# howardlau1999/pytorch-ddp-template

Hardware: AMD Instinct MI355X
Metric: samples/sec (whole node) ResNet-18/CIFAR-shape DDP (higher is better)
Workload: dtype bf16; 1 GPU; model=resnet18-cifar, global_batch=8192, image=32, num_classes=10, parallelism=dp1, hip_graph=True, optimizer=sgd+momentum(master fp32)

## Files before the change

pytorch_ddp_template_amd/ops/csrc/conv_glds.hip:

```cpp

#include <torch/extension.h>

#include "common.h"
#include "dispatch.h"

namespace cg {

typedef __bf16 bf16x8 __attribute__((ext_vector_type(8)));
typedef float f32x4 __attribute__((ext_vector_type(4)));

constexpr int BM = 256, BK = 64;
constexpr int THREADS = 512;

__device__ __forceinline__ f32x4 mfma16(bf16x8 a, bf16x8 b, f32x4 c) {
  return __builtin_amdgcn_mfma_f32_16x16x32_bf16(a, b, c, 0, 0, 0);
}

__device__ __forceinline__ int kswz(int row, int kbyte) {
  return kbyte ^ (((row >> 2) & 1) << 5);
}

struct Geom {
  int H, W, C, lgC, HO, WO, stride, pad, S, RS;
  int lgSt = 0;
};

constexpr int EPI_NONE = 0, EPI_ADD = 1, EPI_MASK = 2, EPI_ADD_MASK = 3;
constexpr int EPI_BNSTATS = 4, EPI_MASK_BNSTATS = EPI_MASK | EPI_BNSTATS;

constexpr int halo_pitch(int hw) { return (hw + 2 + 7) & ~7; }
constexpr int halo_bytes(int hw) {
  return hw ? (BM / hw + 2) * halo_pitch(hw) * BK * 2 : 0;
}

template <int BN, bool STATS, int EPI = EPI_NONE, int HW = 0>
__global__ __launch_bounds__(THREADS, HW ? 4 : BN == 64 ? 2 : 1)
void conv_fwd_glds_kernel(
    const __hip_bfloat16* __restrict__ x, const __hip_bfloat16* __restrict__ w,
    __hip_bfloat16* __restrict__ y, const __hip_bfloat16* __restrict__ zpad,
    int M, int N , int K , Geom g,
    float* __restrict__ stats_ws, int ws_nblocks,
    const __hip_bfloat16* __restrict__ addend,
    const __hip_bfloat16* __restrict__ out_mask,
    const float* __restrict__ bn_mean, const float* __restrict__ bn_rstd) {
  static_assert(!(STATS && EPI != EPI_NONE),
                "dgrad epilogues carry no forward stats");
  static_assert(!(EPI & EPI_BNSTATS) || EPI == EPI_MASK_BNSTATS,
                "BN-backward sums ride only with the mask, without an addend");
  static_assert(HW == 0 || (BN == 64 && BM % HW == 0 && HW % 16 == 0),
                "halo variant: 64-wide tile, whole image rows per M-tile");
  constexpr int HALO_ELEMS = halo_bytes(HW) / 2;
  __shared__ __hip_bfloat16
      smem[HW ? HALO_ELEMS + 2 * BN * BK : 2 * (BM + BN) * BK];

  const int tid = threadIdx.x;
  const int lane = tid & 63;
  const int wave = tid >> 6;

  long long nwg = (long long)gridDim.x * gridDim.y;
  long long bid = (long long)blockIdx.y * gridDim.x + blockIdx.x;
  {
    const long long q = nwg >> 3, r = nwg & 7;
    const int xcd = (int)(bid & 7);
    const long long o = bid >> 3;
    bid = (xcd < r ? xcd * (q + 1) : r * (q + 1) + (xcd - r) * q) + o;
  }
  const int n0 = (int)(bid % gridDim.x) * BN;
  const long long m0 = (bid / gridDim.x) * BM;
  const long long flat_id = bid;

  const int srow = (tid >> 3) & 7;
  const int schunk = lane & 7;
  constexpr int RA = BM / 64;
  constexpr int RB = BN / 64;

  long long nbase[RA];
  int hv[RA], wv[RA];
#pragma unroll
  for (int r = 0; r < RA; ++r) {
    const long long m = m0 + r * 64 + wave * 8 + srow;
    const int wo = (int)(m % g.WO);
    const long long t = m / g.WO;
    const int ho = (int)(t % g.HO);
    const long long n = t / g.HO;
    hv[r] = ho * g.stride - g.pad;
    wv[r] = wo * g.stride - g.pad;
    nbase[r] = n * g.H * (long long)g.W;
  }
  const int smask = (1 << g.lgSt) - 1;

  auto stage = [&](int buf, int kt) {
    __hip_bfloat16* sa = smem + buf * ((BM + BN) * BK);
    __hip_bfloat16* sb = sa + BM * BK;
    const int tap = (kt << 6) >> g.lgC;
    const int c0 = (kt << 6) & (g.C - 1);
    const int rt = tap / g.S, st = tap - rt * g.S;
#pragma unroll
    for (int r = 0; r < RA; ++r) {
      const int row = r * 64 + wave * 8 + srow;
      const int kk = c0 + kswz(row, schunk * 16) / 2;
      const __hip_bfloat16* src = zpad;
      const int hs = hv[r] + rt, ws = wv[r] + st;
      if ((unsigned)(hs >> g.lgSt) < (unsigned)g.H &&
          (unsigned)(ws >> g.lgSt) < (unsigned)g.W &&
          ((hs | ws) & smask) == 0)
        src = x + ((nbase[r] + (long long)(hs >> g.lgSt) * g.W +
                    (ws >> g.lgSt))
                   << g.lgC) +
              kk;
      __builtin_amdgcn_global_load_lds(
          (const __attribute__((address_space(1))) unsigned int*)src,
          (__attribute__((address_space(3))) unsigned int*)(
              sa + (r * 64 + wave * 8) * BK),
          16, 0, 0);
    }
#pragma unroll
    for (int r = 0; r < RB; ++r) {
      const int row = r * 64 + wave * 8 + srow;
      const long long kk = (long long)kt * BK + kswz(row, schunk * 16) / 2;
      __builtin_amdgcn_global_load_lds(
          (const __attribute__((address_space(1))) unsigned int*)(
              w + (long long)(n0 + row) * K + kk),
          (__attribute__((address_space(3))) unsigned int*)(
              sb + (r * 64 + wave * 8) * BK),
          16, 0, 0);
    }
  };

  constexpr int NWM = BM / 128;
  constexpr int NWN = 8 / NWM;
  constexpr int NI = BN / (16 * NWN);
  const int wm = (wave / NWN) * 128;
  const int wn = (wave % NWN) * (NI * 16);
  const int frow = lane & 15;
  const int fkb = (lane >> 4) * 16;

  f32x4 acc[8][NI];
#pragma unroll
  for (int i = 0; i < 8; ++i)
#pragma unroll
    for (int j = 0; j < NI; ++j) acc[i][j] = f32x4{0.f, 0.f, 0.f, 0.f};

  if constexpr (HW == 0) {
    const int NT = K / BK;
    stage(0, 0);
    __syncthreads();

    int cur = 0;
    for (int kt = 0; kt < NT; ++kt) {
      if (kt + 1 < NT) stage(cur ^ 1, kt + 1);
      const __hip_bfloat16* sa = smem + cur * ((BM + BN) * BK);
      const __hip_bfloat16* sb = sa + BM * BK;
      bf16x8 bf[NI][2];
#pragma unroll
      for (int ni = 0; ni < NI; ++ni)
#pragma unroll
        for (int ks = 0; ks < 2; ++ks) {
          const int row = wn + ni * 16 + frow;
          bf[ni][ks] = *(const bf16x8*)((const char*)(sb + row * BK) +
                                        kswz(row, ks * 64 + fkb));
        }
#pragma unroll
      for (int mi = 0; mi < 8; ++mi) {
        bf16x8 af[2];
#pragma unroll
        for (int ks = 0; ks < 2; ++ks) {
          const int row = wm + mi * 16 + frow;
          af[ks] = *(const bf16x8*)((const char*)(sa + row * BK) +
                                    kswz(row, ks * 64 + fkb));
        }
#pragma unroll
        for (int ni = 0; ni < NI; ++ni) {
          acc[mi][ni] = mfma16(af[0], bf[ni][0], acc[mi][ni]);
          acc[mi][ni] = mfma16(af[1], bf[ni][1], acc[mi][ni]);
        }
      }
      __syncthreads();
      cur ^= 1;
    }
  } else {
    constexpr int HP = halo_pitch(HW);
    constexpr int KR = BM / HW;
    constexpr int PPR = HP / 8;
    constexpr int NPIECE = (KR + 2) * PPR;
    __hip_bfloat16* sw = smem + HALO_ELEMS;
    const int tpi = g.H / KR;
    const int tile = (int)(m0 / BM);
    const long long img = tile / tpi;
    const int h0 = (tile - (int)img * tpi) * KR;

    auto stage_w = [&](int buf, int kt) {
      __hip_bfloat16* sb = sw + buf * (BN * BK);
#pragma unroll
      for (int r = 0; r < RB; ++r) {
        const int row = r * 64 + wave * 8 + srow;
        const long long kk = (long long)kt * BK + kswz(row, schunk * 16) / 2;
        __builtin_amdgcn_global_load_lds(
            (const __attribute__((address_space(1))) unsigned int*)(
                w + (long long)(n0 + row) * K + kk),
            (__attribute__((address_space(3))) unsigned int*)(
                sb + (r * 64 + wave * 8) * BK),
            16, 0, 0);
      }
    };
    stage_w(0, 0);
#pragma unroll
    for (int p0 = 0; p0 < NPIECE; p0 += 8) {
      const int pc = p0 + wave;
      if (pc < NPIECE) {
        const int hr = pc / PPR;
        const int hi = h0 - 1 + hr;
        const int wi = (pc - hr * PPR) * 8 + (lane & 7) - 1;
        const __hip_bfloat16* src = zpad;
        if ((unsigned)hi < (unsigned)g.H && (unsigned)wi < (unsigned)HW)
          src = x + (((img * g.H + hi) * HW + wi) << 6) + (lane >> 3) * 8;
        __builtin_amdgcn_global_load_lds(
            (const __attribute__((address_space(1))) unsigned int*)src,
            (__attribute__((address_space(3))) unsigned int*)(smem + pc * 512),
            16, 0, 0);
      }
    }
    int abase[3];
#pragma unroll
    for (int st = 0; st < 3; ++st) {
      const int q = frow + st;
      abase[st] = (wm / HW) * HP * 128 + (q >> 3) * 1024 + (q & 7) * 16 +
                  (lane >> 4) * 128;
    }
    __syncthreads();

#pragma unroll 1
    for (int rt = 0; rt < 3; ++rt)
#pragma unroll
    for (int st = 0; st < 3; ++st) {
      const int kt = rt * 3 + st;
      if (kt + 1 < 9) stage_w((kt + 1) & 1, kt + 1);
      const __hip_bfloat16* sb = sw + (kt & 1) * (BN * BK);
      const char* ha = (const char*)smem + rt * (HP * 128) + abase[st];
      bf16x8 bf[NI][2];
#pragma unroll
      for (int ni = 0; ni < NI; ++ni)
#pragma unroll
        for (int ks = 0; ks < 2; ++ks) {
          const int row = wn + ni * 16 + frow;
          bf[ni][ks] = *(const bf16x8*)((const char*)(sb + row * BK) +
                                        kswz(row, ks * 64 + fkb));
        }
#pragma unroll
      for (int mi = 0; mi < 8; ++mi) {
        const int cpos = ((mi * 16) / HW) * HP + (mi * 16) % HW;
        bf16x8 af[2];
#pragma unroll
        for (int ks = 0; ks < 2; ++ks)
          af[ks] = *(const bf16x8*)(ha + cpos * 128 + ks * 512);
#pragma unroll
        for (int ni = 0; ni < NI; ++ni) {
          acc[mi][ni] = mfma16(af[0], bf[ni][0], acc[mi][ni]);
          acc[mi][ni] = mfma16(af[1], bf[ni][1], acc[mi][ni]);
        }
      }
      __syncthreads();
    }
  }

  if (STATS && stats_ws) {
#pragma unroll
    for (int ni = 0; ni < NI; ++ni) {
      float sv = 0.f, qv = 0.f;
#pragma unroll
      for (int mi = 0; mi < 8; ++mi)
#pragma unroll
        for (int reg = 0; reg < 4; ++reg) {
          const float v = acc[mi][ni][reg];
          sv += v;
          qv += v * v;
        }
      sv += __shfl_xor(sv, 16);
      qv += __shfl_xor(qv, 16);
      sv += __shfl_xor(sv, 32);
      qv += __shfl_xor(qv, 32);
      if (lane < 16) {
        const int col = n0 + wn + ni * 16 + frow;
        const long long wsrow =
            ((flat_id * NWM + wave / NWN)) % ws_nblocks;
        atomicAdd(&stats_ws[wsrow * N + col], sv);
        atomicAdd(&stats_ws[((long long)ws_nblocks + wsrow) * N + col], qv);
      }
    }
  }

  __hip_bfloat16* cs = smem;
  constexpr int CPR = BN / 8;
  constexpr int RPR = THREADS / CPR;
  constexpr int NR = BM / RPR;
  const int wrow = tid / CPR, wchunk = tid % CPR;
  constexpr bool HAS_ADD = (EPI & EPI_ADD) != 0;
  constexpr bool HAS_MASK = (EPI & EPI_MASK) != 0;
  constexpr bool HAS_BNS = (EPI & EPI_BNSTATS) != 0;
  constexpr int PF = 2;
  static_assert(NR >= PF, "epilogue prefetch deeper than the store loop");
  short8 av[PF] = {}, mv[PF] = {};
  auto epi_load = [&](int r, int slot) {
    const long long off =
        ((m0 + r * RPR + wrow) * N + n0) * 2 + wchunk * 16;
    if constexpr (HAS_ADD || HAS_BNS)
      av[slot] = *(const short8*)((const char*)addend + off);
    if constexpr (HAS_MASK)
      mv[slot] = *(const short8*)((const char*)out_mask + off);
  };
  if constexpr (EPI != EPI_NONE) {
#pragma unroll
    for (int p = 0; p < PF; ++p) epi_load(p, p);
  }
#pragma unroll
  for (int mi = 0; mi < 8; ++mi)
#pragma unroll
    for (int ni = 0; ni < NI; ++ni) {
      const int col = wn + ni * 16 + frow;
#pragma unroll
      for (int reg = 0; reg < 4; ++reg) {
        const int row = wm + mi * 16 + (lane >> 4) * 4 + reg;
        cs[row * BN + col] = f2bf(acc[mi][ni][reg]);
      }
    }
  float mu[8] = {}, rs[8] = {}, sdg[8] = {}, sdb[8] = {};
  if constexpr (HAS_BNS) {
#pragma unroll
    for (int j = 0; j < 8; ++j) {
      mu[j] = bn_mean[n0 + wchunk * 8 + j];
      rs[j] = bn_rstd[n0 + wchunk * 8 + j];
    }
  }
  __syncthreads();
  if constexpr (!HAS_BNS) {
#pragma unroll
    for (int r = 0; r < NR; ++r) {
      const int row = r * RPR + wrow;
      short8 c = *(const short8*)((const char*)(cs + row * BN) + wchunk * 16);
      if constexpr (EPI != EPI_NONE) {
        const short8 a = av[r % PF], m = mv[r % PF];
        if (r + PF < NR) epi_load(r + PF, r % PF);
#pragma unroll
        for (int j = 0; j < 8; ++j) {
          short v = c[j];
          if constexpr (HAS_ADD) v = f2bfbits(bfbits2f(v) + bfbits2f(a[j]));
          if constexpr (HAS_MASK)
            v = f2bfbits(bfbits2f(m[j]) > 0.f ? bfbits2f(v) : 0.f);
          c[j] = v;
        }
      }
      *(short8*)((char*)(y + (m0 + row) * N + n0) + wchunk * 16) = c;
    }
  } else {
    static_assert(PF == 2 && NR % PF == 0, "store loop steps by slot pairs");
    auto store_round = [&](int r, int slot) {
      const int row = r * RPR + wrow;
      short8 c = *(const short8*)((const char*)(cs + row * BN) + wchunk * 16);
      const short8 t = av[slot], m = mv[slot];
      if (r + PF < NR) epi_load(r + PF, slot);
#pragma unroll
      for (int j = 0; j < 8; ++j) {
        const float gv = bfbits2f(m[j]) > 0.f ? bfbits2f(c[j]) : 0.f;
        c[j] = f2bfbits(gv);
        sdb[j] += gv;
        sdg[j] += gv * (bfbits2f(t[j]) - mu[j]) * rs[j];
      }
      *(short8*)((char*)(y + (m0 + row) * N + n0) + wchunk * 16) = c;
    };
#pragma unroll 1
    for (int r = 0; r < NR; r += PF) {
      store_round(r, 0);
      store_round(r + 1, 1);
    }
  }

  if constexpr (HAS_BNS) {
    constexpr int P = THREADS / (2 * BN);
    constexpr int RP = RPR / P;
    static_assert(P >= 1 && RP * P == RPR, "column reduction split");
    static_assert((2 * RPR * BN + P * 2 * BN) * sizeof(float) <=
                      sizeof(smem), "reduction buffers exceed the tile LDS");
    float* red = reinterpret_cast<float*>(smem);
    float* red2 = red + 2 * RPR * BN;
    __syncthreads();
#pragma unroll
    for (int j = 0; j < 8; ++j) {
      red[wrow * BN + wchunk * 8 + j] = sdg[j];
      red[(RPR + wrow) * BN + wchunk * 8 + j] = sdb[j];
    }
    __syncthreads();
    const int ci = tid % (2 * BN), part = tid / (2 * BN);
    const int which = ci / BN, col = ci % BN;
    float s = 0.f;
#pragma unroll
    for (int i = 0; i < RP; ++i)
      s += red[(which * RPR + part * RP + i) * BN + col];
    if constexpr (P > 1) {
      red2[part * 2 * BN + ci] = s;
      __syncthreads();
      if (part != 0) return;
      s = red2[ci];
#pragma unroll
      for (int p = 1; p < P; ++p) s += red2[p * 2 * BN + ci];
    }
    const long long wsrow = flat_id % ws_nblocks;
    atomicAdd(&stats_ws[((long long)which * ws_nblocks + wsrow) * N + n0 + col],
              s);
  }
}

}

struct GldsBnStats {
  const torch::Tensor& bn_x;
  const torch::Tensor& mean;
  const torch::Tensor& rstd;
  torch::Tensor ws;
};

constexpr int kBnStatsRows = 1024;

bool conv_halo64_eligible(int64_t H, int64_t W, int64_t C, int64_t Kout,
                          int64_t R, int64_t S, int64_t stride, int64_t pad) {
  if (R != 3 || S != 3 || stride != 1 || pad != 1 || C != 64) return false;
  if (Kout <= 0 || Kout % 64 || Kout % 128 == 0) return false;
  if (W < 16 || W % 16 || cg::BM % W) return false;
  const int64_t k = cg::BM / W;
  if (k > H || H % k) return false;
  return cg::halo_bytes((int)W) + 2 * 64 * cg::BK * 2 <=
         2 * (cg::BM + 64) * cg::BK * 2;
}

static bool conv2d_glds_launch(const torch::Tensor& x, const torch::Tensor& w,
                               torch::Tensor& y, const torch::Tensor& zp,
                               int64_t stride, int64_t pad, float* stats_ws,
                               int ws_nblocks, int lgSt,
                               const c10::optional<torch::Tensor>& addend,
                               const c10::optional<torch::Tensor>& out_mask,
                               GldsBnStats* bns) {
  static const char* e = getenv("PDT_CONV_GLDS");
  if (e && e[0] == '0') return false;
  if (x.scalar_type() != torch::kBFloat16) return false;
  const int N_ = (int)x.size(0), H = (int)x.size(1), W = (int)x.size(2),
            C = (int)x.size(3);
  const int Kout = (int)w.size(0), R = (int)w.size(1), S = (int)w.size(2);
  if (C < 64 || (C & (C - 1))) return false;
  const int HO = (int)y.size(1), WO = (int)y.size(2);
  const int lgC = log2_exact(C);
  const long long M = (long long)N_ * HO * WO;
  const int K = R * S * C;
  if (Kout % 64) return false;
  const int BN = Kout % 256 == 0 ? 256 : Kout % 128 == 0 ? 128 : 64;
  if (M % cg::BM) return false;
  if (M / cg::BM > 2147483647LL / 8) return false;
  cg::Geom g{H, W, C, lgC, HO, WO, (int)stride, (int)pad, S, R * S, lgSt};
  auto stream = c10::hip::getCurrentHIPStream();
  dim3 grid(Kout / BN, (unsigned)(M / cg::BM));
  const int epi = (addend.has_value() ? cg::EPI_ADD : 0) |
                  (out_mask.has_value() ? cg::EPI_MASK : 0);
  for (const auto* t : {&addend, &out_mask}) {
    if (!t->has_value()) continue;
    TORCH_CHECK(!stats_ws,
                "conv glds: addend/out_mask exclude the stats epilogue");
    TORCH_CHECK((*t)->is_cuda() && (*t)->is_contiguous() &&
                    (*t)->scalar_type() == x.scalar_type() &&
                    (*t)->numel() == y.numel(),
                "conv glds: addend/out_mask must be contiguous, of dy's dtype "
                "and dx-sized");
  }
  const bf16* addp = addend.has_value() ? ptr16<bf16>(*addend) : nullptr;
  const bf16* maskp = out_mask.has_value() ? ptr16<bf16>(*out_mask) : nullptr;
  const float *meanp = nullptr, *rstdp = nullptr;
  if (bns) {
    TORCH_CHECK(epi == cg::EPI_MASK && !stats_ws,
                "conv glds: BN-backward sums need out_mask and no addend");
    TORCH_CHECK(bns->bn_x.is_cuda() && bns->bn_x.is_contiguous() &&
                    bns->bn_x.scalar_type() == x.scalar_type() &&
                    bns->bn_x.numel() == y.numel(),
                "conv glds: bn_x must be contiguous, of dy's dtype and "
                "dx-sized");
    for (const auto* t : {&bns->mean, &bns->rstd})
      TORCH_CHECK(t->is_cuda() && t->is_contiguous() &&
                      t->scalar_type() == torch::kFloat32 &&
                      t->numel() == Kout,
                  "conv glds: bn_mean/bn_rstd must be fp32 [C]");
    ws_nblocks = (int)std::min<long long>(kBnStatsRows,
                                          (long long)grid.x * grid.y);
    bns->ws = torch::zeros({2LL * ws_nblocks, Kout},
                           x.options().dtype(torch::kFloat32));
    stats_ws = bns->ws.data_ptr<float>();
    addp = ptr16<bf16>(bns->bn_x);
    meanp = bns->mean.data_ptr<float>();
    rstdp = bns->rstd.data_ptr<float>();
  }
  const char* eh = getenv("PDT_CONV_HALO64");
  const bool halo = !(eh && eh[0] == '0') && lgSt == 0 && H == HO && W == WO &&
                    conv_halo64_eligible(H, W, C, Kout, R, S, stride, pad);
#define CG_HALO(ST, EP)                                       \
  (W == 16   ? &cg::conv_fwd_glds_kernel<64, ST, EP, 16>      \
   : W == 32 ? &cg::conv_fwd_glds_kernel<64, ST, EP, 32>      \
             : &cg::conv_fwd_glds_kernel<64, ST, EP, 64>)
#define CG_KERN(ST, EP)                                       \
  (halo        ? CG_HALO(ST, EP)                              \
   : BN == 256 ? &cg::conv_fwd_glds_kernel<256, ST, EP>       \
   : BN == 128 ? &cg::conv_fwd_glds_kernel<128, ST, EP>       \
               : &cg::conv_fwd_glds_kernel<64, ST, EP>)
  auto kern = bns                     ? CG_KERN(false, cg::EPI_MASK_BNSTATS)
              : stats_ws              ? CG_KERN(true, cg::EPI_NONE)
              : epi == cg::EPI_NONE   ? CG_KERN(false, cg::EPI_NONE)
              : epi == cg::EPI_ADD    ? CG_KERN(false, cg::EPI_ADD)
              : epi == cg::EPI_MASK   ? CG_KERN(false, cg::EPI_MASK)
                                      : CG_KERN(false, cg::EPI_ADD_MASK);
#undef CG_KERN
#undef CG_HALO
  hipLaunchKernelGGL(kern, grid, dim3(cg::THREADS), 0, stream, ptr16<bf16>(x),
                     ptr16<bf16>(w), ptr16<bf16>(y), ptr16<bf16>(zp), (int)M,
                     Kout, K, g, stats_ws, ws_nblocks, addp, maskp, meanp,
                     rstdp);
  return true;
}

bool conv2d_fwd_glds_ex(const torch::Tensor& x, const torch::Tensor& w,
                        torch::Tensor& y, const torch::Tensor& zp,
                        int64_t stride, int64_t pad, float* stats_ws,
                        int ws_nblocks, int lgSt,
                        const c10::optional<torch::Tensor>& addend,
                        const c10::optional<torch::Tensor>& out_mask) {
  return conv2d_glds_launch(x, w, y, zp, stride, pad, stats_ws, ws_nblocks,
                            lgSt, addend, out_mask, nullptr);
}

torch::Tensor conv2d_dgrad_glds_bnstats(
    const torch::Tensor& dy, const torch::Tensor& wr, torch::Tensor& dx,
    const torch::Tensor& zp, int64_t pad, int lgSt,
    const torch::Tensor& out_mask, const torch::Tensor& bn_x,
    const torch::Tensor& bn_mean, const torch::Tensor& bn_rstd) {
  GldsBnStats bns{bn_x, bn_mean, bn_rstd, torch::Tensor()};
  if (!conv2d_glds_launch(dy, wr, dx, zp, 1, pad, nullptr, 0, lgSt,
                          c10::nullopt, out_mask, &bns))
    return torch::Tensor();
  return bns.ws;
}

bool conv2d_fwd_glds(const torch::Tensor& x, const torch::Tensor& w,
                     torch::Tensor& y, const torch::Tensor& zp,
                     int64_t stride, int64_t pad, float* stats_ws,
                     int ws_nblocks) {
  return conv2d_fwd_glds_ex(x, w, y, zp, stride, pad, stats_ws, ws_nblocks,
                            0, c10::nullopt, c10::nullopt);
}
```

pytorch_ddp_template_amd/ops/csrc/ops.cpp:

```cpp

#include <torch/extension.h>

#include <vector>

torch::Tensor relu_fwd(torch::Tensor x);
torch::Tensor relu_bwd(torch::Tensor dy, torch::Tensor y);
torch::Tensor add_relu_fwd(torch::Tensor a, torch::Tensor b);
torch::Tensor add_(torch::Tensor a, torch::Tensor b);
torch::Tensor gelu_fwd(torch::Tensor x);
torch::Tensor gelu_bwd(torch::Tensor dy, torch::Tensor x);
torch::Tensor col_sum(torch::Tensor dy);
torch::Tensor transpose2d(torch::Tensor x);
torch::Tensor avgpool_global(torch::Tensor x);
torch::Tensor avgpool_global_bwd(torch::Tensor dy, int64_t H, int64_t W);
std::vector<torch::Tensor> maxpool2d_fwd(torch::Tensor x, int64_t k, int64_t s,
                                         int64_t p);
torch::Tensor maxpool2d_bwd(torch::Tensor dy, torch::Tensor idx, int64_t H,
                            int64_t W);
torch::Tensor weight_rot(torch::Tensor w);
torch::Tensor zero_stuff(torch::Tensor dy, int64_t s, int64_t opad_h,
                         int64_t opad_w);
torch::Tensor im2col(torch::Tensor x, int64_t R, int64_t S, int64_t stride,
                     int64_t pad, int64_t Kpad);
torch::Tensor bmm_nt_bf16(torch::Tensor A, torch::Tensor B,
                          c10::optional<torch::Tensor> bias, bool relu);
torch::Tensor gemm_nt_splitk_f32(torch::Tensor A, torch::Tensor B);
torch::Tensor bmm_tn_bf16(torch::Tensor A, torch::Tensor B);
std::vector<torch::Tensor> bmm_tn_bias_bf16(torch::Tensor A, torch::Tensor B);
torch::Tensor conv2d_fwd_bf16(torch::Tensor x, torch::Tensor w,
                              c10::optional<torch::Tensor> bias, int64_t stride,
                              int64_t pad, bool relu);
torch::Tensor conv2d_wgrad_bf16(torch::Tensor dy, torch::Tensor x,
                                int64_t stride, int64_t pad, int64_t R,
                                int64_t S);
torch::Tensor conv2d_dgrad_bf16(torch::Tensor dy, torch::Tensor wr,
                                int64_t stride, int64_t pad, int64_t H,
                                int64_t W,
                                c10::optional<torch::Tensor> addend,
                                c10::optional<torch::Tensor> addend_mask,
                                c10::optional<torch::Tensor> out_mask);
std::vector<torch::Tensor> conv2d_fwd_stats_bf16(
    torch::Tensor x, torch::Tensor w, c10::optional<torch::Tensor> bias,
    int64_t stride, int64_t pad, bool relu);
std::vector<torch::Tensor> conv2d_dgrad_bnstats_bf16(
    torch::Tensor dy, torch::Tensor wr, int64_t stride, int64_t pad, int64_t H,
    int64_t W, torch::Tensor out_mask, torch::Tensor bn_x,
    torch::Tensor bn_mean, torch::Tensor bn_rstd);
bool conv_halo64_eligible(int64_t H, int64_t W, int64_t C, int64_t Kout,
                          int64_t R, int64_t S, int64_t stride, int64_t pad);
torch::Tensor bmm_nt_f32(torch::Tensor A, torch::Tensor B,
                         c10::optional<torch::Tensor> bias, bool relu);
torch::Tensor bmm_tn_f32(torch::Tensor A, torch::Tensor B);
torch::Tensor conv2d_fwd_f32(torch::Tensor x, torch::Tensor w,
                             c10::optional<torch::Tensor> bias, int64_t stride,
                             int64_t pad, bool relu);
torch::Tensor conv2d_wgrad_f32(torch::Tensor dy, torch::Tensor x,
                               int64_t stride, int64_t pad, int64_t R,
                               int64_t S);
std::vector<torch::Tensor> bn_fwd(torch::Tensor x, torch::Tensor gamma,
                                  torch::Tensor beta,
                                  c10::optional<torch::Tensor> running_mean,
                                  c10::optional<torch::Tensor> running_var,
                                  double momentum, double eps, bool relu);
std::vector<torch::Tensor> bn_fwd_ws(torch::Tensor x, torch::Tensor gamma,
                                     torch::Tensor beta, torch::Tensor ws,
                                     c10::optional<torch::Tensor> running_mean,
                                     c10::optional<torch::Tensor> running_var,
                                     double momentum, double eps, bool relu,
                                     c10::optional<torch::Tensor> addend);
torch::Tensor bn_infer(torch::Tensor x, torch::Tensor gamma, torch::Tensor beta,
                       torch::Tensor rmean, torch::Tensor rvar, double eps,
                       bool relu);
std::vector<torch::Tensor> bn_bwd(torch::Tensor dy, torch::Tensor x,
                                  torch::Tensor gamma, torch::Tensor mean,
                                  torch::Tensor rstd,
                                  c10::optional<torch::Tensor> y_relu);
std::vector<torch::Tensor> bn_bwd_ws(torch::Tensor dy, torch::Tensor x,
                                     torch::Tensor gamma, torch::Tensor mean,
                                     torch::Tensor rstd, torch::Tensor ws);
std::vector<torch::Tensor> layernorm_fwd(torch::Tensor x, torch::Tensor gamma,
                                         torch::Tensor beta, double eps);
std::vector<torch::Tensor> layernorm_bwd(torch::Tensor dy, torch::Tensor x,
                                         torch::Tensor gamma,
                                         torch::Tensor mean,
                                         torch::Tensor rstd);
torch::Tensor softmax_fwd(torch::Tensor x, double scale);
torch::Tensor softmax_bwd(torch::Tensor dy, torch::Tensor y, double scale);
std::vector<torch::Tensor> ce_fwd(torch::Tensor logits, torch::Tensor target);
torch::Tensor ce_bwd(torch::Tensor logits, torch::Tensor target,
                     torch::Tensor lse, torch::Tensor dloss);
torch::Tensor mse_fwd(torch::Tensor p, torch::Tensor t);
torch::Tensor mse_bwd(torch::Tensor p, torch::Tensor t, torch::Tensor dloss);
std::vector<torch::Tensor> qkv_unpack(torch::Tensor qkv, int64_t heads);
torch::Tensor qkv_pack(torch::Tensor dq, torch::Tensor dk, torch::Tensor dv,
                       int64_t N, int64_t heads);
torch::Tensor head_split(torch::Tensor x, int64_t heads);
std::vector<torch::Tensor> attn_fwd(torch::Tensor qkv, int64_t heads,
                                    double scale, bool want_p);
torch::Tensor attn_bwd(torch::Tensor qkv, torch::Tensor dout,
                       torch::Tensor out, torch::Tensor stats, int64_t heads,
                       double scale);
void sgd_step(std::vector<torch::Tensor> params,
              std::vector<torch::Tensor> grads,
              std::vector<torch::Tensor> moms,
              std::vector<torch::Tensor> masters, double lr, double momentum,
              double wd, double damp, bool nesterov,
              c10::optional<torch::Tensor> guard,
              c10::optional<torch::Tensor> skip_count,
              c10::optional<torch::Tensor> lr_tensor);
torch::Tensor l2norm_sq(std::vector<torch::Tensor> grads);
void scale_(std::vector<torch::Tensor> ts, double s);
void scale_by_tensor_(std::vector<torch::Tensor> ts, torch::Tensor s);


namespace {

bool is_bf16(const torch::Tensor& t) {
  return t.scalar_type() == torch::kBFloat16 ||
         t.scalar_type() == torch::kHalf;
}

int k_granule(const torch::Tensor& t) { return is_bf16(t) ? 8 : 4; }

torch::Tensor pad_k(const torch::Tensor& t, int mult) {
  long long K = t.size(-1);
  long long pad = (mult - K % mult) % mult;
  if (pad == 0) return t;
  return torch::constant_pad_nd(t, {0, pad});
}

bool pow2_ge(int v, int lo) {
  return v >= lo && (v & (v - 1)) == 0;
}

}

torch::Tensor gemm_nt(torch::Tensor A, torch::Tensor B,
                      c10::optional<torch::Tensor> bias, bool relu,
                      bool ) {
  TORCH_CHECK(A.scalar_type() == B.scalar_type(), "dtype mismatch");
  int g = k_granule(A);
  if (A.size(-1) % g) {
    A = pad_k(A.contiguous(), g);
    B = pad_k(B.contiguous(), g);
  }
  if (is_bf16(A)) return bmm_nt_bf16(A.contiguous(), B.contiguous(), bias, relu);
  return bmm_nt_f32(A.contiguous(), B.contiguous(), bias, relu);
}

torch::Tensor gemm_tn(torch::Tensor A, torch::Tensor B) {
  if (is_bf16(A)) return bmm_tn_bf16(A.contiguous(), B.contiguous());
  return bmm_tn_f32(A.contiguous(), B.contiguous());
}

torch::Tensor bmm_nt(torch::Tensor A, torch::Tensor B) {
  int g = k_granule(A);
  if (A.size(-1) % g) {
    A = pad_k(A.contiguous(), g);
    B = pad_k(B.contiguous(), g);
  }
  if (is_bf16(A)) return bmm_nt_bf16(A.contiguous(), B.contiguous(), {}, false);
  return bmm_nt_f32(A.contiguous(), B.contiguous(), {}, false);
}

torch::Tensor bmm_tn(torch::Tensor A, torch::Tensor B) {
  auto C = is_bf16(A) ? bmm_tn_bf16(A.contiguous(), B.contiguous())
                      : bmm_tn_f32(A.contiguous(), B.contiguous());
  return C.to(A.scalar_type());
}

torch::Tensor bmm_nn(torch::Tensor A, torch::Tensor B) {
  auto Bt = transpose2d(B.contiguous());
  return bmm_nt(A, Bt);
}


torch::Tensor conv2d_fwd(torch::Tensor x, torch::Tensor w,
                         c10::optional<torch::Tensor> bias, int64_t stride,
                         int64_t pad, bool relu) {
  int Cin = (int)x.size(3);
  int R = (int)w.size(1), S = (int)w.size(2), Kout = (int)w.size(0);
  const bool fast = is_bf16(x) ? pow2_ge(Cin, 8) : pow2_ge(Cin, 4);
  if (fast) {
    if (is_bf16(x))
      return conv2d_fwd_bf16(x.contiguous(), w.contiguous(), bias, stride, pad,
                             relu);
    return conv2d_fwd_f32(x.contiguous(), w.contiguous(), bias, stride, pad,
                          relu);
  }
  int K = R * S * Cin;
  int g = k_granule(x);
  int Kpad = (K + g - 1) / g * g;
  auto cols = im2col(x.contiguous(), R, S, stride, pad, Kpad);
  auto wf = pad_k(w.contiguous().reshape({Kout, K}), g);
  auto y = is_bf16(x) ? bmm_nt_bf16(cols, wf.contiguous(), bias, relu)
                      : bmm_nt_f32(cols, wf.contiguous(), bias, relu);
  int N = (int)x.size(0), H = (int)x.size(1), W = (int)x.size(2);
  int HO = (H + 2 * (int)pad - R) / (int)stride + 1;
  int WO = (W + 2 * (int)pad - S) / (int)stride + 1;
  return y.reshape({N, HO, WO, Kout});
}

torch::Tensor conv2d_dgrad(torch::Tensor dy, torch::Tensor w, int64_t stride,
                           int64_t pad, int64_t H, int64_t W,
                           c10::optional<torch::Tensor> addend,
                           c10::optional<torch::Tensor> addend_mask,
                           c10::optional<torch::Tensor> out_mask) {
  int R = (int)w.size(1), S = (int)w.size(2);
  TORCH_CHECK(pad <= R - 1 && pad <= S - 1, "dgrad needs pad <= kernel-1");
  auto wr = weight_rot(w.contiguous());
  int Kout = (int)dy.size(3);
  if (is_bf16(dy) ? pow2_ge(Kout, 8) : false) {
    return conv2d_dgrad_bf16(dy.contiguous(), wr, stride, pad, H, W, addend,
                             addend_mask, out_mask);
  }
  int64_t opad_h = (H + 2 * pad - R) % stride;
  int64_t opad_w = (W + 2 * pad - S) % stride;
  auto dys = stride > 1 ? zero_stuff(dy.contiguous(), stride, opad_h, opad_w)
                        : dy.contiguous();
  auto dx = conv2d_fwd(dys, wr, {}, 1, R - 1 - pad, false);
  if (addend.has_value()) {
    auto a = *addend;
    if (addend_mask.has_value())
      a = a * (addend_mask->reshape(a.sizes()) > 0).to(a.scalar_type());
    dx = dx + a.reshape(dx.sizes());
  }
  if (out_mask.has_value())
    dx = torch::where(out_mask->reshape(dx.sizes()) > 0, dx,
                      torch::zeros_like(dx));
  TORCH_CHECK(dx.size(1) == H && dx.size(2) == W,
              "dgrad shape mismatch: got ", dx.sizes(), " want H=", H, " W=",
              W, " (input H+2p-R must be divisible by stride)");
  return dx;
}

std::tuple<torch::Tensor, c10::optional<torch::Tensor>> conv2d_dgrad_bnstats(
    torch::Tensor dy, torch::Tensor w, int64_t stride, int64_t pad, int64_t H,
    int64_t W, torch::Tensor out_mask, torch::Tensor bn_x,
    torch::Tensor bn_mean, torch::Tensor bn_rstd) {
  int R = (int)w.size(1), S = (int)w.size(2);
  TORCH_CHECK(pad <= R - 1 && pad <= S - 1, "dgrad needs pad <= kernel-1");
  if (is_bf16(dy) && pow2_ge((int)dy.size(3), 8)) {
    auto wr = weight_rot(w.contiguous());
    auto r = conv2d_dgrad_bnstats_bf16(dy.contiguous(), wr, stride, pad, H, W,
                                       out_mask, bn_x, bn_mean, bn_rstd);
    if (r.size() == 2) return {r[0], r[1]};
    return {r[0], c10::nullopt};
  }
  return {conv2d_dgrad(dy, w, stride, pad, H, W, c10::nullopt, c10::nullopt,
                       out_mask),
          c10::nullopt};
}

torch::Tensor conv2d_wgrad(torch::Tensor dy, torch::Tensor x, int64_t stride,
                           int64_t pad, int64_t R, int64_t S) {
  int Cin = (int)x.size(3);
  const bool fast = is_bf16(x) ? pow2_ge(Cin, 8) : pow2_ge(Cin, 4);
  dy = dy.contiguous();
  x = x.contiguous();
  if (fast) {
    return is_bf16(x) ? conv2d_wgrad_bf16(dy, x, stride, pad, R, S)
                      : conv2d_wgrad_f32(dy, x, stride, pad, R, S);
  }
  int K = (int)(R * S * Cin);
  int g = k_granule(x);
  int Kpad = (K + g - 1) / g * g;
  auto cols = im2col(x, R, S, stride, pad, Kpad);
  int Kout = (int)dy.size(3);
  auto dw = is_bf16(x)
                ? bmm_tn_bf16(dy.reshape({-1, Kout}).contiguous(), cols)
                : bmm_tn_f32(dy.reshape({-1, Kout}).contiguous(), cols);
  return dw.narrow(1, 0, K).reshape({Kout, R, S, Cin}).contiguous();
}

PYBIND11_MODULE(TORCH_EXTENSION_NAME, m) {
  m.def("gemm_nt", &gemm_nt, py::arg("A"), py::arg("B"),
        py::arg("bias") = c10::nullopt, py::arg("relu") = false,
        py::arg("out_f32") = false);
  m.def("gemm_tn", &gemm_tn);
  m.def("gemm_nt_splitk_f32", &gemm_nt_splitk_f32);
  m.def("gemm_tn_bias", [](torch::Tensor A, torch::Tensor B) {
    TORCH_CHECK(A.scalar_type() == torch::kBFloat16 ||
                A.scalar_type() == torch::kHalf,
                "gemm_tn_bias: 16-bit dtypes only");
    return bmm_tn_bias_bf16(A.contiguous(), B.contiguous());
  });
  m.def("bmm_nt", &bmm_nt);
  m.def("bmm_nn", &bmm_nn);
  m.def("bmm_tn", &bmm_tn);
  m.def("transpose2d", &transpose2d);
  m.def("conv2d_fwd", &conv2d_fwd, py::arg("x"), py::arg("w"),
        py::arg("bias") = c10::nullopt, py::arg("stride") = 1,
        py::arg("pad") = 0, py::arg("relu") = false);
  m.def("conv2d_dgrad", &conv2d_dgrad, py::arg("dy"), py::arg("w"),
        py::arg("stride"), py::arg("pad"), py::arg("H"), py::arg("W"),
        py::arg("addend") = c10::nullopt,
        py::arg("addend_mask") = c10::nullopt,
        py::arg("out_mask") = c10::nullopt);
  m.def("conv2d_dgrad_bnstats", &conv2d_dgrad_bnstats, py::arg("dy"),
        py::arg("w"), py::arg("stride"), py::arg("pad"), py::arg("H"),
        py::arg("W"), py::arg("out_mask"), py::arg("bn_x"),
        py::arg("bn_mean"), py::arg("bn_rstd"));
  m.def("conv2d_fwd_stats", &conv2d_fwd_stats_bf16, py::arg("x"),
        py::arg("w"), py::arg("bias") = c10::nullopt, py::arg("stride") = 1,
        py::arg("pad") = 0, py::arg("relu") = false);
  m.def("conv_halo64_eligible", &conv_halo64_eligible, py::arg("H"),
        py::arg("W"), py::arg("C"), py::arg("Kout"), py::arg("R"),
        py::arg("S"), py::arg("stride"), py::arg("pad"));
  m.def("conv2d_wgrad", &conv2d_wgrad);
  m.def("relu_fwd", &relu_fwd);
  m.def("relu_bwd", &relu_bwd);
  m.def("add_relu_fwd", &add_relu_fwd);
  m.def("add_", &add_);
  m.def("gelu_fwd", &gelu_fwd);
  m.def("gelu_bwd", &gelu_bwd);
  m.def("col_sum", &col_sum);
  m.def("avgpool_global", &avgpool_global);
  m.def("avgpool_global_bwd", &avgpool_global_bwd);
  m.def("maxpool2d_fwd", &maxpool2d_fwd);
  m.def("maxpool2d_bwd", &maxpool2d_bwd);
  m.def("bn_fwd", &bn_fwd);
  m.def("bn_fwd_ws", &bn_fwd_ws, py::arg("x"), py::arg("gamma"),
        py::arg("beta"), py::arg("ws"), py::arg("running_mean"),
        py::arg("running_var"), py::arg("momentum"), py::arg("eps"),
        py::arg("relu"), py::arg("addend") = c10::nullopt);
  m.def("bn_infer", &bn_infer);
  m.def("bn_bwd", &bn_bwd, py::arg("dy"), py::arg("x"), py::arg("gamma"),
        py::arg("mean"), py::arg("rstd"), py::arg("y_relu") = c10::nullopt);
  m.def("bn_bwd_ws", &bn_bwd_ws, py::arg("dy"), py::arg("x"),
        py::arg("gamma"), py::arg("mean"), py::arg("rstd"), py::arg("ws"));
  m.def("layernorm_fwd", &layernorm_fwd);
  m.def("layernorm_bwd", &layernorm_bwd);
  m.def("softmax_fwd", &softmax_fwd);
  m.def("attn_fwd", &attn_fwd, py::arg("qkv"), py::arg("heads"),
        py::arg("scale"), py::arg("want_p") = false);
  m.def("attn_bwd", &attn_bwd);
  m.def("qkv_unpack", &qkv_unpack);
  m.def("qkv_pack", &qkv_pack);
  m.def("head_split", &head_split);
  m.def("softmax_bwd", &softmax_bwd);
  m.def("ce_fwd", &ce_fwd);
  m.def("ce_bwd", &ce_bwd);
  m.def("mse_fwd", &mse_fwd);
  m.def("mse_bwd", &mse_bwd);
  m.def("sgd_step", &sgd_step, py::arg("params"), py::arg("grads"),
        py::arg("moms"), py::arg("masters"), py::arg("lr"),
        py::arg("momentum"), py::arg("wd"), py::arg("damp"),
        py::arg("nesterov"), py::arg("guard") = py::none(),
        py::arg("skip_count") = py::none(),
        py::arg("lr_tensor") = py::none());
  m.def("l2norm_sq", &l2norm_sq);
  m.def("scale_", &scale_);
  m.def("scale_by_tensor_", &scale_by_tensor_);
  m.def("im2col", &im2col);
  m.def("weight_rot", &weight_rot);
  m.def("zero_stuff", &zero_stuff);
}
```

Baseline: 143,200 samples/sec.

## Split stride-2 dgrad into output-parity classes to skip zero-dilated taps

Adds a parity-split variant of the implicit-GEMM conv kernel for the data-gradient of 3x3 stride-2 convolutions. Each M-tile handles one (row, column) output parity class and gathers only the 1, 2 or 4 taps that touch real (non-dilated) input, instead of iterating all 9 taps and loading zero padding for most of them. Output rows are scattered back to interleaved positions in the epilogue. This cuts wasted MFMA and load work by roughly half or more for stride-2 dgrad layers. The cost is load imbalance across parity tiles and strided epilogue stores. It is enabled by default and can be turned off with an env var.

```diff
diff --git a/pytorch_ddp_template_amd/ops/csrc/conv_glds.hip b/pytorch_ddp_template_amd/ops/csrc/conv_glds.hip
--- a/pytorch_ddp_template_amd/ops/csrc/conv_glds.hip
+++ b/pytorch_ddp_template_amd/ops/csrc/conv_glds.hip
@@ -33,7 +33,7 @@
   return hw ? (BM / hw + 2) * halo_pitch(hw) * BK * 2 : 0;
 }
 
-template <int BN, bool STATS, int EPI = EPI_NONE, int HW = 0>
+template <int BN, bool STATS, int EPI = EPI_NONE, int HW = 0, bool PAR = false>
 __global__ __launch_bounds__(THREADS, HW ? 4 : BN == 64 ? 2 : 1)
 void conv_fwd_glds_kernel(
     const __hip_bfloat16* __restrict__ x, const __hip_bfloat16* __restrict__ w,
@@ -49,6 +49,8 @@
                 "BN-backward sums ride only with the mask, without an addend");
   static_assert(HW == 0 || (BN == 64 && BM % HW == 0 && HW % 16 == 0),
                 "halo variant: 64-wide tile, whole image rows per M-tile");
+  static_assert(!PAR || (!STATS && HW == 0),
+                "parity split: dgrad only, per-tap gather");
   constexpr int HALO_ELEMS = halo_bytes(HW) / 2;
   __shared__ __hip_bfloat16
       smem[HW ? HALO_ELEMS + 2 * BN * BK : 2 * (BM + BN) * BK];
@@ -66,7 +68,11 @@
     bid = (xcd < r ? xcd * (q + 1) : r * (q + 1) + (xcd - r) * q) + o;
   }
   const int n0 = (int)(bid % gridDim.x) * BN;
-  const long long m0 = (bid / gridDim.x) * BM;
+  const long long mtile = bid / gridDim.x;
+  const int pa = PAR ? (int)(mtile >> 1) & 1 : 0;
+  const int pb = PAR ? (int)mtile & 1 : 0;
+  const long long m0 = (PAR ? mtile >> 2 : mtile) * BM;
+  const int lgH = PAR ? 31 - __clz(g.H) : 0, lgW = PAR ? 31 - __clz(g.W) : 0;
   const long long flat_id = bid;
 
   const int srow = (tid >> 3) & 7;
@@ -79,6 +85,12 @@
 #pragma unroll
   for (int r = 0; r < RA; ++r) {
     const long long m = m0 + r * 64 + wave * 8 + srow;
+    if constexpr (PAR) {
+      hv[r] = (int)(m >> lgW) & (g.H - 1);
+      wv[r] = (int)m & (g.W - 1);
+      nbase[r] = m;
+      continue;
+    }
     const int wo = (int)(m % g.WO);
     const long long t = m / g.WO;
     const int ho = (int)(t % g.HO);
@@ -92,8 +104,14 @@
   auto stage = [&](int buf, int kt) {
     __hip_bfloat16* sa = smem + buf * ((BM + BN) * BK);
     __hip_bfloat16* sb = sa + BM * BK;
-    const int tap = (kt << 6) >> g.lgC;
+    int tap = (kt << 6) >> g.lgC;
     const int c0 = (kt << 6) & (g.C - 1);
+    const int dh = pb ? tap >> 1 : tap, dw = pb ? tap & 1 : 0;
+    int wkt = kt;
+    if constexpr (PAR) {
+      tap = (pa ? 2 * dh : 1) * 3 + (pb ? 2 * dw : 1);
+      wkt = (tap << (g.lgC - 6)) + (c0 >> 6);
+    }
     const int rt = tap / g.S, st = tap - rt * g.S;
 #pragma unroll
     for (int r = 0; r < RA; ++r) {
@@ -101,7 +119,10 @@
       const int kk = c0 + kswz(row, schunk * 16) / 2;
       const __hip_bfloat16* src = zpad;
       const int hs = hv[r] + rt, ws = wv[r] + st;
-      if ((unsigned)(hs >> g.lgSt) < (unsigned)g.H &&
+      if constexpr (PAR) {
+        if (hv[r] + dh < g.H && wv[r] + dw < g.W)
+          src = x + ((nbase[r] + dh * g.W + dw) << g.lgC) + kk;
+      } else if ((unsigned)(hs >> g.lgSt) < (unsigned)g.H &&
           (unsigned)(ws >> g.lgSt) < (unsigned)g.W &&
           ((hs | ws) & smask) == 0)
         src = x + ((nbase[r] + (long long)(hs >> g.lgSt) * g.W +
@@ -117,7 +138,7 @@
 #pragma unroll
     for (int r = 0; r < RB; ++r) {
       const int row = r * 64 + wave * 8 + srow;
-      const long long kk = (long long)kt * BK + kswz(row, schunk * 16) / 2;
+      const long long kk = (long long)wkt * BK + kswz(row, schunk * 16) / 2;
       __builtin_amdgcn_global_load_lds(
           (const __attribute__((address_space(1))) unsigned int*)(
               w + (long long)(n0 + row) * K + kk),
@@ -142,7 +163,7 @@
     for (int j = 0; j < NI; ++j) acc[i][j] = f32x4{0.f, 0.f, 0.f, 0.f};
 
   if constexpr (HW == 0) {
-    const int NT = K / BK;
+    const int NT = PAR ? ((1 + pa) * (1 + pb)) << (g.lgC - 6) : K / BK;
     stage(0, 0);
     __syncthreads();
 
@@ -300,9 +321,19 @@
   constexpr int PF = 2;
   static_assert(NR >= PF, "epilogue prefetch deeper than the store loop");
   short8 av[PF] = {}, mv[PF] = {};
+  auto yrow = [&](int row) -> long long {
+    if constexpr (PAR) {
+      const long long m = m0 + row;
+      const int i = (int)(m >> lgW) & (g.H - 1), j = (int)m & (g.W - 1);
+      return ((((m >> (lgW + lgH)) << (lgH + 1)) + 2 * i + pa) << (lgW + 1)) +
+             2 * j + pb;
+    } else {
+      return m0 + row;
+    }
+  };
   auto epi_load = [&](int r, int slot) {
     const long long off =
-        ((m0 + r * RPR + wrow) * N + n0) * 2 + wchunk * 16;
+        (yrow(r * RPR + wrow) * N + n0) * 2 + wchunk * 16;
     if constexpr (HAS_ADD || HAS_BNS)
       av[slot] = *(const short8*)((const char*)addend + off);
     if constexpr (HAS_MASK)
@@ -349,7 +380,7 @@
           c[j] = v;
         }
       }
-      *(short8*)((char*)(y + (m0 + row) * N + n0) + wchunk * 16) = c;
+      *(short8*)((char*)(y + yrow(row) * N + n0) + wchunk * 16) = c;
     }
   } else {
     static_assert(PF == 2 && NR % PF == 0, "store loop steps by slot pairs");
@@ -365,7 +396,7 @@
         sdb[j] += gv;
         sdg[j] += gv * (bfbits2f(t[j]) - mu[j]) * rs[j];
       }
-      *(short8*)((char*)(y + (m0 + row) * N + n0) + wchunk * 16) = c;
+      *(short8*)((char*)(y + yrow(row) * N + n0) + wchunk * 16) = c;
     };
 #pragma unroll 1
     for (int r = 0; r < NR; r += PF) {
@@ -429,6 +460,20 @@
   if (k > H || H % k) return false;
   return cg::halo_bytes((int)W) + 2 * 64 * cg::BK * 2 <=
          2 * (cg::BM + 64) * cg::BK * 2;
+}
+
+bool conv_dgrad_s2_parity_eligible(int64_t H, int64_t W, int64_t Cin,
+                                   int64_t Kout, int64_t R, int64_t S,
+                                   int64_t stride, int64_t pad, int64_t N) {
+  if (R != 3 || S != 3 || stride != 2 || pad != 1) return false;
+  if (N <= 0 || H <= 0 || W <= 0 || (H & 1) || (W & 1)) return false;
+  const int64_t HO = H / 2, WO = W / 2;
+  if ((HO & (HO - 1)) || (WO & (WO - 1))) return false;
+  if (Kout < 64 || (Kout & (Kout - 1))) return false;
+  if (Cin <= 0 || Cin % 64) return false;
+  const int64_t Mc = N * HO * WO;
+  if (Mc % cg::BM) return false;
+  return 4 * (Mc / cg::BM) <= 2147483647LL / 8;
 }
 
 static bool conv2d_glds_launch(const torch::Tensor& x, const torch::Tensor& w,
@@ -505,12 +550,23 @@
    : BN == 256 ? &cg::conv_fwd_glds_kernel<256, ST, EP>       \
    : BN == 128 ? &cg::conv_fwd_glds_kernel<128, ST, EP>       \
                : &cg::conv_fwd_glds_kernel<64, ST, EP>)
-  auto kern = bns                     ? CG_KERN(false, cg::EPI_MASK_BNSTATS)
+  const char* ep = getenv("PDT_DGRAD_S2_PARITY");
+  const bool par = !(ep && ep[0] == '0') && lgSt == 1 && stride == 1 &&
+                   (bns || !stats_ws) && HO == 2 * H && WO == 2 * W &&
+                   conv_dgrad_s2_parity_eligible(HO, WO, Kout, C, R, S, 2,
+                                                 R - 1 - pad, N_);
+#define CG_DGRAD(EP)                                                      \
+  (!par        ? CG_KERN(false, EP)                                       \
+   : BN == 256 ? &cg::conv_fwd_glds_kernel<256, false, EP, 0, true>       \
+   : BN == 128 ? &cg::conv_fwd_glds_kernel<128, false, EP, 0, true>       \
+               : &cg::conv_fwd_glds_kernel<64, false, EP, 0, true>)
+  auto kern = bns                     ? CG_DGRAD(cg::EPI_MASK_BNSTATS)
               : stats_ws              ? CG_KERN(true, cg::EPI_NONE)
-              : epi == cg::EPI_NONE   ? CG_KERN(false, cg::EPI_NONE)
-              : epi == cg::EPI_ADD    ? CG_KERN(false, cg::EPI_ADD)
-              : epi == cg::EPI_MASK   ? CG_KERN(false, cg::EPI_MASK)
-                                      : CG_KERN(false, cg::EPI_ADD_MASK);
+              : epi == cg::EPI_NONE   ? CG_DGRAD(cg::EPI_NONE)
+              : epi == cg::EPI_ADD    ? CG_DGRAD(cg::EPI_ADD)
+              : epi == cg::EPI_MASK   ? CG_DGRAD(cg::EPI_MASK)
+                                      : CG_DGRAD(cg::EPI_ADD_MASK);
+#undef CG_DGRAD
 #undef CG_KERN
 #undef CG_HALO
   hipLaunchKernelGGL(kern, grid, dim3(cg::THREADS), 0, stream, ptr16<bf16>(x),
diff --git a/pytorch_ddp_template_amd/ops/csrc/ops.cpp b/pytorch_ddp_template_amd/ops/csrc/ops.cpp
--- a/pytorch_ddp_template_amd/ops/csrc/ops.cpp
+++ b/pytorch_ddp_template_amd/ops/csrc/ops.cpp
@@ -48,6 +48,9 @@
     torch::Tensor bn_mean, torch::Tensor bn_rstd);
 bool conv_halo64_eligible(int64_t H, int64_t W, int64_t C, int64_t Kout,
                           int64_t R, int64_t S, int64_t stride, int64_t pad);
+bool conv_dgrad_s2_parity_eligible(int64_t H, int64_t W, int64_t Cin,
+                                   int64_t Kout, int64_t R, int64_t S,
+                                   int64_t stride, int64_t pad, int64_t N);
 torch::Tensor bmm_nt_f32(torch::Tensor A, torch::Tensor B,
                          c10::optional<torch::Tensor> bias, bool relu);
 torch::Tensor bmm_tn_f32(torch::Tensor A, torch::Tensor B);
@@ -307,6 +310,10 @@
   m.def("conv_halo64_eligible", &conv_halo64_eligible, py::arg("H"),
         py::arg("W"), py::arg("C"), py::arg("Kout"), py::arg("R"),
         py::arg("S"), py::arg("stride"), py::arg("pad"));
+  m.def("conv_dgrad_s2_parity_eligible", &conv_dgrad_s2_parity_eligible,
+        py::arg("H"), py::arg("W"), py::arg("Cin"), py::arg("Kout"),
+        py::arg("R"), py::arg("S"), py::arg("stride"), py::arg("pad"),
+        py::arg("N"));
   m.def("conv2d_wgrad", &conv2d_wgrad);
   m.def("relu_fwd", &relu_fwd);
   m.def("relu_bwd", &relu_bwd);
```

Result: faster. 148,900 samples/sec (median of 6 runs) (+4.0%).
